# qinjr/SCoRe

Hardware: AMD Instinct MI355X
Metric: train samples/sec @ batch=1024 (higher is better)
Workload: dtype f32

## Files before the change

score_amd/csrc/engine.hip:

```cpp
#include <string.h>
#include <stdlib.h>
#include <stdio.h>
#include <math.h>
#include <mutex>
#include <new>
#include "common.h"
#include "kernels.h"
#include "persample.h"

namespace {

const int FC1 = 200, FC2 = 80, AT1 = 80, AT2 = 40;
const int CASER_L = SCORE_CASER_L, CASER_HPAD = SCORE_CASER_HPAD;
const int MAX_ENTRIES = 48;

enum Family { FAM_SLICE, FAM_GCMC, FAM_G4R, FAM_CASER, FAM_DELF, FAM_DEEMS, FAM_SVDPP, FAM_SASREC };

struct Dims {
  int64_t N;
  int D, H, T, K, Fu, Fi, mt;
  int Du, Di, I, Dq, NI, Dk, Dhead, nstate;
  int Is[2];
  bool coattn, attn;
  Family family;
  int n_gru;
  bool fc_head;
  bool sums_1hop;
  bool reads_targets;
  int Ic;
  int off_u, off_i, off_ti, off_tu;
};
// ... 221 lines not shown
static inline bool same_key(const LayoutKey& a, const LayoutKey& b) { return memcmp(&a, &b, sizeof(a)) == 0; }
int build_layout(const Dims& d, score_param_entry_t* out, int max_entries, Params* P) {
  struct Memo { bool ok; LayoutKey k; Params P; int n; score_param_entry_t ent[MAX_ENTRIES]; };
  static thread_local Memo memo = {};
  LayoutKey k = layout_key(d, 0);
  if (!memo.ok || !same_key(memo.k, k)) {
    memset(&memo.k, 0, sizeof(memo.k));
    memo.n = build_layout_raw(d, memo.ent, MAX_ENTRIES, &memo.P);
    memo.k = k; memo.ok = memo.n >= 0;
    if (memo.n < 0) return memo.n;
  }
  *P = memo.P;
  if (out) {
    if (memo.n > max_entries) return SCORE_E_BADARG;
    memcpy(out, memo.ent, sizeof(score_param_entry_t) * memo.n);
  }
  return memo.n;
}

struct WS {
  int64_t xside[2], info, rsave[2], query, head_inp, att_score, logit, y_pred, loss;
  int64_t gru_out[2], gru_final[2], xproj[2], gates[2];
  int64_t q, ainp, a1, a2, bn, f1, f2, lossb, dlogit, part;
  int64_t weff, wq, qz, adzsum, dweff, dwq, dqd;
  int64_t dwslab, dwslab_floats, dgstage, scratch2, gru_tmp, gru_tmp_floats;
  int64_t dz2, dz1, dbn, dhead, ds, da2, da1, dainp, dgru[2], dinfo, dq, dquery, dfinal[2];
  int64_t dxproj[2], rh[2], hprev[2], dxside[2], dzsum[2], S, scratch;
  int64_t pcoef[2], dzcoef[2], dtgt, keys_in, keys_out, vals_in, vals_out, sort_temp, partials;
  int64_t n_occ, sort_temp_bytes, partial_floats;
  int64_t uid, unique_rows, meta, remap[6];
  int64_t ca_slab, ca_slab_floats, cs_part, cs_part_floats, wxcat;
  int64_t pimg_x[2], pimg_d[2];
  int64_t psimg;
  int64_t gcmc_a[2], gcmc_z[2], gcmc_dz[2], gcmc_da[2], gcmc_pn, gcmc_g, gcmc_gu;
  int64_t caser_hwin, caser_arg, caser_v;
  int64_t delf_key[2], delf_att[2], delf_rep[2], delf_ds[2], delf_dpre[2], delf_act, delf_dact;
  int64_t deems_f1, deems_f2, deems_dz1, deems_dz2, deems_logit, deems_y, deems_dlogit;
  int64_t svdpp_act, svdpp_dw;
  int64_t sas_nrm, sas_qin, sas_q, sas_k, sas_v, sas_y, sas_dq, sas_dk, sas_dv, sas_rstd, sas_km, sas_p, sas_att, sas_fin,
      sas_dgamma, sas_dbeta, sas_hin, sas_dhin, sas_z1, sas_dz1, sas_f1, sas_dz1e, sas_z2, sas_f2, sas_dz2, sas_logit, sas_dlogit;
  int64_t scratch_floats, total;
};

static int panel_x_splits(int H) { return 3 * H <= 512 ? 1 : ((3 * H) % 32 == 0 && 3 * H <= 1024 ? 2 : 0); }
static int panel_d_splits(int I) { return I <= 512 ? 1 : (I % 32 == 0 && I <= 1024 ? 2 : 0); }

static int64_t ps_image_region_floats(const Dims& d) {
  if (d.H != 32 || !d.coattn || !d.attn) return 0;
  PsShape s;
  memset(&s, 0, sizeof(s));
  s.H = d.H; s.I = d.I; s.Dk = d.Dk; s.Dhead = d.Dhead;
  PsImages im;
  ps_plan_images(s, &im);
  return im.total;
}

static inline int64_t weff_copy_stride(const Dims& d) { return align_up64(2 * (int64_t)d.Dk * AT1 + 48, 4); }
struct Taker {
  int64_t cur;
  int64_t operator()(int64_t n) { int64_t o = cur; cur = align_up64(cur + (n > 0 ? n : 4), 4); return o; }
};
void ws_family_regions(const Dims& d, int B, Taker& take, WS* w) {
  const int64_t BT = (int64_t)B * d.T;
  if (d.family == FAM_GCMC) {
    const int Dx[2] = {d.Di, d.Du};
    for (int s = 0; s < 2; ++s) {
      w->gcmc_a[s] = take(BT * Dx[s]); w->gcmc_z[s] = take(BT * Dx[s]);
      w->gcmc_dz[s] = take(BT * Dx[s]); w->gcmc_da[s] = take(BT * Dx[s]);
    }
    w->gcmc_pn = take(2 * (int64_t)B * d.H); w->gcmc_g = take(B); w->gcmc_gu = take(2 * (int64_t)B * d.H);
  } else {
    for (int s = 0; s < 2; ++s) w->gcmc_a[s] = w->gcmc_z[s] = w->gcmc_dz[s] = w->gcmc_da[s] = -1;
    w->gcmc_pn = w->gcmc_g = w->gcmc_gu = -1;
  }
  if (d.family == FAM_CASER) {
    w->caser_hwin = take((int64_t)B * (d.T - CASER_L + 1)); w->caser_arg = take(B); w->caser_v = take((int64_t)B * d.Di);
  } else {
    w->caser_hwin = w->caser_arg = w->caser_v = -1;
  }
  if (d.family == FAM_DELF) {
// ... 31 lines not shown
  } else {
    w->sas_nrm = w->sas_qin = w->sas_q = w->sas_k = w->sas_v = w->sas_y = w->sas_dq = w->sas_dk = w->sas_dv = w->sas_rstd = w->sas_km =
        w->sas_p = w->sas_att = w->sas_fin = w->sas_dgamma = w->sas_dbeta = w->sas_hin = w->sas_dhin = w->sas_z1 = w->sas_dz1 = w->sas_f1 =
            w->sas_dz1e = w->sas_z2 = w->sas_f2 = w->sas_dz2 = w->sas_logit = w->sas_dlogit = -1;
  }
}

void build_ws_raw(const Dims& d, int B, WS* w) {
  Taker take = {0};
  const int64_t BT = (int64_t)B * d.T;
  for (int s = 0; s < 2; ++s) w->xside[s] = take(BT * d.I);
  w->info = take(BT * 4 * d.K);
  for (int c = 0; c < 2; ++c) w->rsave[c] = take(BT * d.K);
  w->query = take((int64_t)B * d.Dq);
  w->head_inp = take((int64_t)B * d.Dhead);
  w->att_score = take(BT);
  w->logit = take(B); w->y_pred = take(B); w->loss = take(4);
  for (int s = 0; s < 2; ++s) w->gru_out[s] = take(BT * d.H);
  for (int s = 0; s < 2; ++s) w->gru_final[s] = take((int64_t)B * d.H);
  for (int s = 0; s < 2; ++s) w->xproj[s] = take(BT * 3 * d.H);
  for (int s = 0; s < 2; ++s) w->gates[s] = take(BT * 3 * d.H);
  w->q = take((int64_t)B * d.Dk);
  w->ainp = take(BT * 2 * d.Dk);
  w->weff = take(SCORE_WEFF_COPIES * weff_copy_stride(d)); w->wq = take((int64_t)d.Dk * AT1); w->qz = take((int64_t)B * AT1);
  w->a1 = take(BT * AT1); w->a2 = take(BT * AT2);
  w->bn = take((int64_t)B * d.Dhead);
  w->f1 = take((int64_t)B * FC1); w->f2 = take((int64_t)B * FC2);
  w->lossb = take(B); w->dlogit = take(B); w->part = take(256 + 4);
  w->dz2 = take((int64_t)B * FC2); w->dz1 = take((int64_t)B * FC1);
  w->dbn = take((int64_t)B * d.Dhead); w->dhead = take((int64_t)B * d.Dhead);
  w->ds = take(BT); w->da2 = take(BT * AT2); w->da1 = take(BT * AT1);
  w->dainp = take(BT * 2 * d.Dk);
  w->adzsum = take((int64_t)B * AT1); w->dweff = take(2 * (int64_t)d.Dk * AT1); w->dwq = take((int64_t)d.Dk * AT1);
  w->dqd = take((int64_t)B * d.Dk);
  for (int s = 0; s < 2; ++s) w->dgru[s] = take(BT * d.H);
  w->dinfo = take(BT * 4 * d.K);
  w->dq = take((int64_t)B * d.Dk); w->dquery = take((int64_t)B * d.Dq);
  for (int s = 0; s < 2; ++s) w->dfinal[s] = take((int64_t)B * d.H);
  for (int s = 0; s < 2; ++s) {
    w->dxproj[s] = take(BT * 3 * d.H);
    w->rh[s] = take(BT * d.H);
    w->hprev[s] = take(BT * d.H + 3 * (int64_t)d.H * d.H);
  }
  for (int s = 0; s < 2; ++s) w->dxside[s] = take(BT * d.I);
  for (int c = 0; c < 2; ++c) w->dzsum[c] = take(BT);
  w->S = take(2 * (int64_t)B);
  w->scratch_floats = 4 << 20;
// ... 164 lines not shown
  return 0;
}

#define G(call) SCORE_TRY(call)
static inline int gemm_mode_call(int x3, int tr, int M, int N, int K, const float* A, int lda, const float* B,
                                 int ldb, float* C, int ldc, const float* bias, int flags, float keep,
                                 const uint8_t* mask, uint64_t seed, float* scratch, int64_t scratch_floats,
                                 void* s) {
  return score_gemm(tr, M, N, K, A, lda, B, ldb, C, ldc, bias, flags | x3, keep, mask, seed, scratch, scratch_floats,
                    s);
}
#define EV(i) \
  do { if (stage_events && stage_events[i]) HIPTRY(hipEventRecord((hipEvent_t)stage_events[i], s)); } while (0)

static inline uint32_t clamp_rows(int64_t n) { return (uint32_t)(n < 0x80000000ll ? n : 0x80000000ll); }
static inline int global_batch(const score_state_t* st, int B) { return st->global_batch > 0 ? st->global_batch : B; }

struct Pass {
  Dims d; Params P; WS w; Flags fl;
  const score_state_t* st; const score_batch_t* bt;
  int B, T, BT, H;
  int x3, Bg;
  uint32_t n_rows;
  int64_t weff_stride;
  float rs;
  float* ws; const float* W; float* scratch;
  hipStream_t s;
};
static int pass_fill(Pass* c, const score_state_t* st, const score_batch_t* bt, void* stream) {
  const Dims& d = c->d;
  build_layout(d, nullptr, 0, &c->P);
  c->st = st; c->bt = bt; c->fl = flags_of(st);
  c->B = bt->B; c->T = active_T(d, bt); c->H = d.H; c->BT = c->B * c->T;
  build_ws(d, c->B, &c->w);
  if (c->w.total * 4 > st->workspace_bytes) return SCORE_E_WORKSPACE;
  c->x3 = st->gemm_mode == 1 ? GF_X3 : 0; c->Bg = global_batch(st, c->B); c->n_rows = clamp_rows(st->n_table_rows);
  c->weff_stride = weff_copy_stride(d); c->rs = (float)(1.0 / sqrt(1.0 + 1e-3));
  c->ws = st->workspace; c->W = st->w; c->scratch = c->ws + c->w.scratch;
  c->s = (hipStream_t)stream;
  return 0;
}
static inline const float* wxcat(const Pass& c, int sd) { return c.ws + c.w.wxcat + (int64_t)sd * (c.d.Ic + 1) * 3 * c.H; }
static int weight_prep(const Pass& c, hipStream_t on) {
  const Dims& d = c.d; const Params& P = c.P; const WS& w = c.w; const float* W = c.W;
  return score_launch_weight_prep(W + P.gk[0], W + P.ck[0], W + P.gb[0], W + P.cb[0], W + P.gk[1], W + P.ck[1], W + P.gb[1],
                                  W + P.cb[1], d.Is[0], d.Is[1], d.Ic, d.H, c.ws + w.wxcat, d.Dk, AT1,
                                  d.attn ? W + P.at_w[1] : nullptr, c.ws + w.weff, c.ws + w.wq, SCORE_WEFF_COPIES, c.weff_stride, W,
                                  P.n_reg, c.ws + w.part, on);
}

static inline const float* gru_x_rows(const Pass& c, int sd) {
  return c.ws + (c.d.family == FAM_GCMC ? c.w.gcmc_z[sd] : (c.d.family == FAM_G4R && sd == 1) ? c.w.gru_out[0] : c.w.xside[sd]);
}

static void gru_header(const Pass& c, GruArgs* ga) {
  memset(ga, 0, sizeof(*ga));
  ga->B = c.B; ga->T = c.T; ga->H = c.H; ga->length = c.bt->length;
  ga->nw8 = 1;
  ga->tmp = c.ws + c.w.gru_tmp; ga->tmp_floats = c.w.gru_tmp_floats;
  ga->x3 = c.x3 != 0; ga->x3_rec = ga->x3 && !c.fl.gru_f32_rec; ga->stepwise = c.fl.gru_stepwise;
}
static void gru_side(const Pass& c, int sd, GruSide* g) {
  const int H = c.H;
  g->Wg = c.W + c.P.gk[sd] + (int64_t)c.d.Is[sd] * 2 * H; g->ldwg = 2 * H;
  g->Wc = c.W + c.P.ck[sd] + (int64_t)c.d.Is[sd] * H; g->ldwc = H;
  g->out = c.ws + c.w.gru_out[sd]; g->ldo = H; g->gates = c.ws + c.w.gates[sd];
}
static void gru_side_saved(const Pass& c, int sd, GruSide* g) {
  g->dxproj = c.ws + c.w.dxproj[sd]; g->rh = c.ws + c.w.rh[sd]; g->hprev = c.ws + c.w.hprev[sd];
}
// ... 825 lines not shown
      G(panel_launch(c, 0, xin, xp));
    } else {
      const float* Bx[2] = {wxcat(c, 0), wxcat(c, 1)};
      const float* bx[2] = {Bx[0] + (int64_t)d.Is[0] * 3 * H, Bx[1] + (int64_t)d.Is[1] * 3 * H};
      G(score_gemm_same_shape(0, 2, BT, 3 * H, d.Is[0], xin, x_ld(d, 0), Bx, 3 * H, xp, 3 * H, GF_BIAS, x3 != 0, c.scratch,
                              w.scratch_floats, s, bx));
    }
  }
  for (int sd = 0; sd < 2; ++sd) {
    const float* cat = wxcat(c, sd);
    if (d.Is[0] != d.Is[1])
      G(gemm_mode_call(x3, 0, BT, 3 * H, d.Is[sd], xin[sd], x_ld(d, sd), cat, 3 * H, xp[sd], 3 * H, cat + (int64_t)d.Is[sd] * 3 * H,
                       GF_BIAS, 1.f, nullptr, 0, c.scratch, w.scratch_floats, s));
    gru_side(c, sd, &ga.s[sd]);
    ga.s[sd].xproj = xp[sd]; ga.s[sd].final_state = ws + w.gru_final[sd];
  }
  return score_gru_fwd_multi(ga, 2, s);
}

int fwd_attention(const Pass& c, const FwdState& f) {
  const Dims& d = c.d; const Params& P = c.P; const WS& w = c.w; const score_batch_t* bt = c.bt;
  float* ws = c.ws; const float* W = c.W; const int B = c.B, T = c.T, H = c.H, BT = c.BT, x3 = c.x3; hipStream_t s = c.s;
  HIPTRY(hipStreamWaitEvent(s, f.sd->join, 0));
  int frc = c.fl.attn_unfused ? SCORE_E_SHAPE
                : score_launch_attn_fwd_fused(B, T, H, d.NI, AT1, AT2, ws + w.q, ws + w.gru_out[0], ws + w.gru_out[1],
                                              ws + w.info, ws + w.weff, ws + w.qz, W + P.at_w[2], W + P.at_b[2],
                                              W + P.at_w[3], W + P.at_b[3], bt->length, ws + w.ainp, ws + w.a1, ws + w.a2,
                                              ws + w.att_score, ws + w.head_inp, d.Dhead, d.off_u, d.off_i, s,
                                              SCORE_WEFF_COPIES, c.weff_stride);
  if (frc != SCORE_E_SHAPE) return frc;
  G(score_launch_attn_build_inp(B, T, H, d.NI, ws + w.q, ws + w.gru_out[0], ws + w.gru_out[1], ws + w.info,
                                ws + w.ainp, s));
  G(gemm_mode_call(x3, 0, BT, AT1, 2 * d.Dk, ws + w.ainp, 2 * d.Dk, ws + w.weff, AT1, ws + w.a1, AT1, ws + w.qz,
                   GF_BIAS | GF_RELU | (T << 16), 1.f, nullptr, 0, c.scratch, w.scratch_floats, s));
  int trc = c.fl.attn_unfused ? SCORE_E_SHAPE
                : score_launch_attn_tail_fwd(B, T, H, AT1, AT2, ws + w.a1, W + P.at_w[2], W + P.at_b[2], W + P.at_w[3],
                                             W + P.at_b[3], bt->length, ws + w.gru_out[0], ws + w.gru_out[1], ws + w.a2,
                                             ws + w.att_score, ws + w.head_inp, d.Dhead, d.off_u, d.off_i, s);
  if (trc != SCORE_E_SHAPE) return trc;
  G(gemm_mode_call(x3, 0, BT, AT2, AT1, ws + w.a1, AT1, W + P.at_w[2], AT2, ws + w.a2, AT2, W + P.at_b[2],
                   GF_BIAS | GF_RELU, 1.f, nullptr, 0, c.scratch, w.scratch_floats, s));
  return score_launch_attn_pool_fwd(B, T, H, AT2, ws + w.a2, W + P.at_w[3], W + P.at_b[3], bt->length,
                                    ws + w.gru_out[0], ws + w.gru_out[1], ws + w.att_score, ws + w.head_inp, d.Dhead,
                                    d.off_u, d.off_i, s);
}

int fwd_fc_head(const Pass& c, const FwdState& f) {
  const Dims& d = c.d; const Params& P = c.P; const WS& w = c.w; const score_state_t* st = c.st; const score_batch_t* bt = c.bt;
  float* ws = c.ws; const float* W = c.W; const int B = c.B, x3 = c.x3; hipStream_t s = c.s;
  const float keep_prob = f.keep_prob;
  const int dflag = keep_prob < 1.f ? GF_DROP : 0;
  int hrc = c.fl.head_unfused ? SCORE_E_SHAPE
// ... 664 lines not shown
```

score_amd/csrc/head.hip:

```cpp
#include <stdlib.h>
#include "common.h"
#include "kernels.h"
#include "cell.h"

__device__ __forceinline__ void attn_fold_w1_body(int blk, int Dk, int NA, const float* __restrict__ W1, float* __restrict__ weff,
                                                  float* __restrict__ wq, int copies, int64_t copy_stride) {
  int i = blk * 256 + threadIdx.x;
  if (i >= Dk * NA) return;
  const float wa = W1[i], wb = W1[Dk * NA + i], wc = W1[2 * Dk * NA + i], wd = W1[3 * Dk * NA + i];
  for (int c = 0; c < copies; ++c) {
    weff[c * copy_stride + i] = wb - wc;
    weff[c * copy_stride + Dk * NA + i] = wd;
  }
  wq[i] = wa + wc;
}

__global__ void attn_build_inp_kernel(int BT, int T, int H, int NI, const float* __restrict__ q,
                                      const float* __restrict__ ur, const float* __restrict__ ir,
                                      const float* __restrict__ info, float* __restrict__ inp) {
  const int Dk = 2 * H + NI;
  int64_t i = (int64_t)blockIdx.x * blockDim.x + threadIdx.x;
  if (i >= (int64_t)BT * Dk) return;
  int bt = (int)(i / Dk), j = (int)(i - (int64_t)bt * Dk);
  int b = bt / T;
  float k = j < H ? ur[(int64_t)bt * H + j]
                  : (j < 2 * H ? ir[(int64_t)bt * H + (j - H)] : info[(int64_t)bt * NI + (j - 2 * H)]);
  float qq = q[(int64_t)b * Dk + j];
  float* o = inp + (int64_t)bt * 2 * Dk;
  o[j] = k;
  o[Dk + j] = qq * k;
}
__global__ __launch_bounds__(256) void attn_build_inp4_kernel(int BT, int T, int H, int NI, const float* __restrict__ q,
                                                              const float* __restrict__ ur, const float* __restrict__ ir,
                                                              const float* __restrict__ info, float* __restrict__ inp) {
  const int Dk = 2 * H + NI, Dk4 = Dk >> 2;
  const unsigned i = blockIdx.x * blockDim.x + threadIdx.x;
  if (i >= (unsigned)BT * (unsigned)Dk4) return;
// ... 452 lines not shown
  const float* gk1; const float* ck1; const float* gb1; const float* cb1;
  int I0, I1, Imax, H; float* cat;
};
__device__ __forceinline__ void gru_wxcat_body(int blk, const WxcatArgs& a) {
  const int H = a.H;
  const int64_t per = (int64_t)(a.Imax + 1) * 3 * H;
  int64_t i = (int64_t)blk * 256 + threadIdx.x;
  if (i >= 2 * per) return;
  const int sd = i >= per;
  const int64_t l = i - sd * per;
  const int r = (int)(l / (3 * H)), j = (int)(l - (int64_t)r * 3 * H);
  const int I = sd ? a.I1 : a.I0;
  if (r > I) return;
  const float* gk = sd ? a.gk1 : a.gk0; const float* ck = sd ? a.ck1 : a.ck0;
  const float* gb = sd ? a.gb1 : a.gb0; const float* cb = sd ? a.cb1 : a.cb0;
  float v;
  if (r < I) v = j < 2 * H ? gk[(int64_t)r * 2 * H + j] : ck[(int64_t)r * H + (j - 2 * H)];
  else v = j < 2 * H ? gb[j] : cb[j - 2 * H];
  a.cat[i] = v;
}

struct WeightPrepArgs {
  WxcatArgs wx; int b_wx;
  int Dk, NA; const float* W1; float* weff; float* wq; int copies; int64_t copy_stride; int b_fold;
  const float* wreg; int64_t n_reg; float* part;
};
__global__ __launch_bounds__(256) void weight_prep_kernel(const WeightPrepArgs a) {
  const int b = blockIdx.x;
  if (b < a.b_wx) gru_wxcat_body(b, a.wx);
  else if (b < a.b_wx + a.b_fold) attn_fold_w1_body(b - a.b_wx, a.Dk, a.NA, a.W1, a.weff, a.wq, a.copies, a.copy_stride);
  else sumsq_stage1_body(b - a.b_wx - a.b_fold, L2_PARTS, a.wreg, a.n_reg, a.part);
}
int score_launch_weight_prep(const float* gk0, const float* ck0, const float* gb0, const float* cb0, const float* gk1,
                             const float* ck1, const float* gb1, const float* cb1, int I0, int I1, int Imax, int H, float* cat,
                             int Dk, int NA, const float* W1, float* weff, float* wq, int copies, int64_t copy_stride,
                             const float* wreg, int64_t n_reg, float* part, hipStream_t s) {
  WeightPrepArgs a;
  a.wx = WxcatArgs{gk0, ck0, gb0, cb0, gk1, ck1, gb1, cb1, I0, I1, Imax, H, cat};
  a.b_wx = (int)cdiv64(2 * (int64_t)(Imax + 1) * 3 * H, 256);
  a.Dk = Dk; a.NA = NA; a.W1 = W1; a.weff = weff; a.wq = wq; a.copies = copies; a.copy_stride = copy_stride;
  a.b_fold = W1 ? (Dk * NA + 255) / 256 : 0;
  a.wreg = wreg; a.n_reg = n_reg; a.part = part;
  hipLaunchKernelGGL(weight_prep_kernel, dim3(a.b_wx + a.b_fold + L2_PARTS), dim3(256), 0, s, a);
  SCORE_CHECK_LAUNCH();
  return 0;
}
#define adam1 score_adam1
__global__ void adam_kernel(float* __restrict__ p, float* __restrict__ m, float* __restrict__ v,
                            const float* __restrict__ g, int64_t n4, int64_t n, int64_t n_reg, float l2, float alpha,
                            float omb1, float omb2, float eps, const float* __restrict__ alpha_dev,
                            const int32_t* __restrict__ guard, int32_t* __restrict__ skipped) {
  if (guard && *guard) {
    if (skipped && blockIdx.x == 0 && threadIdx.x == 0) atomicAdd(skipped, 1);
    return;
  }
  if (alpha_dev) alpha = *alpha_dev;
  score_adam_dense_body(p, m, v, g, n4, n, n_reg, l2, alpha, omb1, omb2, eps, (int)blockIdx.x, (int)gridDim.x);
}

#ifndef ADAM_NT
#define ADAM_NT 0
#endif
__device__ __forceinline__ float4 adam_ld(const float* p) {
#if ADAM_NT
  const score_v4f t = __builtin_nontemporal_load(reinterpret_cast<const score_v4f*>(p));
  return make_float4(t.x, t.y, t.z, t.w);
// ... 222 lines not shown
```

score_amd/csrc/head_fused.hip:

```cpp
#include "common.h"
#include "kernels.h"
#include "cell.h"
#include "head_tiles.h"

namespace {

struct HeadFwdArgs {
  int B, Dh, N1, N2, Bglobal;
  const float* x; const float* gamma; const float* beta; float rs;
  const float* W1; const float* b1; const float* W2; const float* b2; const float* W3; const float* b3;
  float keep; int drop; const uint8_t* mask0; const uint8_t* mask1; uint64_t seed0, seed1;
  const uint64_t* seed_dev;
  const int32_t* label;
  float* bn; float* f1; float* f2; float* logit; float* y; float* lossb; float* dlogit;
  float* dz2;
  int phase;
};

__global__ __launch_bounds__(64 * HF_NW) void head_fwd_fused_kernel(const HeadFwdArgs a) {
  extern __shared__ float sm[];
  const uint64_t seed0 = a.seed_dev ? *a.seed_dev : a.seed0;
  const uint64_t seed1 = a.seed_dev ? (seed0 ^ 0x5DEECE66Dull) : a.seed1;
  const int Dh = a.Dh, N1 = a.N1, N2 = a.N2;
  const int Kp0 = (Dh + 15) & ~15, LD0 = Kp0 + 4;
  const int Kp1 = (N1 + 15) & ~15, LD1 = Kp1 + 4;
  const int Kp2 = (N2 + 15) & ~15, LD2 = Kp2 + 4;
// ... 138 lines not shown
      a.y[row] = p;
      a.lossb[row] = logloss_term(p, lab);
      const float dl = logloss_dlogit(p, lab, a.Bglobal);
      a.dlogit[row] = dl;
      xs[i] = dl;
    }
  }
  __syncthreads();
  if (a.dz2) {
    for (int e = tid; e < HF_ROWS * N2; e += 64 * HF_NW) {
      const int i = e / N2, n = e - i * N2, row = b0 + i;
      const float q = xs[i] * a.W3[n] / a.keep;
      if (row < a.B) a.dz2[(int64_t)row * N2 + n] = f2s[i * LD2 + n] > 0.f ? q : 0.f;
    }
  }
}


constexpr int AF_NW = 8;

struct AttnFwdArgs {
  int B, T, H, NI, N1, N2, S;
  const float* q; const float* ur; const float* ir; const float* info;
  const float* Weff; const float* qz;
  const float* W4; const float* b4; const float* w5; const float* b5; const int32_t* length;
  float* inp; float* a1; float* a2; float* score; float* head; int ldh, off_u, off_i;
  int wcopies; int64_t wstride;
};

__device__ __forceinline__ void af_build(const AttnFwdArgs& a, float* __restrict__ xs, int LD, int Kp, int row0,
                                         int row_end, int t0, int nthr) {
  const int Dk = 2 * a.H + a.NI, Dk4 = Dk >> 2, K2 = 2 * Dk;
  const int total = 16 * Dk4;
  constexpr int U = 4;
  for (int e0 = t0; e0 < total; e0 += U * nthr) {
    float4 k[U], qq[U];
    int ii[U], jj[U], gg[U];
    bool ok[U];
#pragma unroll
    for (int u = 0; u < U; ++u) {
      const int e = e0 + u * nthr;
      const int ec = e < total ? e : 0;
      ii[u] = ec / Dk4; jj[u] = (ec - ii[u] * Dk4) * 4;
      gg[u] = row0 + ii[u];
      ok[u] = e < total && gg[u] < row_end;
      const int g = gg[u] < row_end ? gg[u] : row_end - 1;
      const int j = jj[u];
      const float* src = j < a.H ? a.ur + (int64_t)g * a.H + j
                                 : (j < 2 * a.H ? a.ir + (int64_t)g * a.H + (j - a.H) : a.info + (int64_t)g * a.NI + (j - 2 * a.H));
      k[u] = ld4(src);
// ... 10 lines not shown
#endif
      } else {
        kk = make_float4(0.f, 0.f, 0.f, 0.f); qk = kk;
      }
      *reinterpret_cast<float4*>(xs + ii[u] * LD + jj[u]) = kk;
      *reinterpret_cast<float4*>(xs + ii[u] * LD + Dk + jj[u]) = qk;
    }
  }
  for (int e = t0; e < 16 * (Kp - K2); e += nthr) {
    const int i = e / (Kp - K2), j = e - i * (Kp - K2);
    xs[i * LD + K2 + j] = 0.f;
  }
}

template <int KQ>
__global__ __launch_bounds__(64 * AF_NW) void attn_fwd_fused_kernel(const AttnFwdArgs a) {
  extern __shared__ float sm[];
  const int T = a.T, H = a.H, N1 = a.N1, N2 = a.N2;
  const int Dk = 2 * H + a.NI, K2 = 2 * Dk, Kp = 4 * KQ, LD = Kp + 4;
  const int L1 = N1 + 1, L2 = N2 + 1;
  float* xs0 = sm;
  float* xs1 = xs0 + 16 * LD;
  float* a1s = xs1 + 16 * LD;
  float* w4s = a1s + a.S * T * L1;
  float* a2s = w4s + N1 * N2;
  float* scs = a2s + a.S * T * L2;
  const int tid = threadIdx.x, lane = tid & 63, wave = tid >> 6;
  const int lc = lane & 15, lq = lane >> 4;
  const int b0 = blockIdx.x * a.S;
  const int ns = min(a.S, a.B - b0);
  const int row0 = b0 * T, row_end = row0 + ns * T;
  const int ntile = (ns * T + 15) >> 4;
  const int ntn = (N1 + 15) >> 4;

  float breg[KQ];
  if (wave < ntn) {
    const int col = wave * 16 + lc;
    const float* Wsrc = a.Weff + (int64_t)((blockIdx.x >> 3) % a.wcopies) * a.wstride;
#pragma unroll
    for (int s_ = 0; s_ < KQ; ++s_) {
      const int k = lq * KQ + s_;
#ifdef AFP_NOPRELOAD
      const float w = (float)(k + col) * 1e-3f;
#else
      const float w = Wsrc[(int64_t)(k < K2 ? k : K2 - 1) * N1 + (col < N1 ? col : N1 - 1)];
#endif
      breg[s_] = w * ((k < K2 && col < N1) ? 1.0f : 0.0f);
    }
  }
  for (int i = tid; i < N1 * N2; i += 64 * AF_NW) w4s[i] = a.W4[i];
  af_build(a, xs0, LD, Kp, row0, row_end, tid, 64 * AF_NW);
  __syncthreads();
  for (int m = 0; m < ntile; ++m) {
    float* xs = (m & 1) ? xs1 : xs0;
    if (wave < ntn) {
      hf_f32x4 acc[1] = {{0.f, 0.f, 0.f, 0.f}};
      const int n0[1] = {wave * 16};
      const float* xrow = xs + lc * LD + lq * KQ;
#ifndef AFP_NOMFMA
#ifdef AFP_TWOACC
      hf_f32x4 acc2 = {0.f, 0.f, 0.f, 0.f};
#pragma unroll
      for (int s4 = 0; s4 < KQ; s4 += 4) {
        const float4 av = *reinterpret_cast<const float4*>(xrow + s4);
        acc[0] = __builtin_amdgcn_mfma_f32_16x16x4f32(av.x, breg[s4 + 0], acc[0], 0, 0, 0);
        acc2 = __builtin_amdgcn_mfma_f32_16x16x4f32(av.y, breg[s4 + 1], acc2, 0, 0, 0);
        acc[0] = __builtin_amdgcn_mfma_f32_16x16x4f32(av.z, breg[s4 + 2], acc[0], 0, 0, 0);
        acc2 = __builtin_amdgcn_mfma_f32_16x16x4f32(av.w, breg[s4 + 3], acc2, 0, 0, 0);
      }
      acc[0] += acc2;
// ... 27 lines not shown
#endif
          }
        }
      }
    } else if (m + 1 < ntile) {
#ifndef AFP_NOBUILD
      af_build(a, (m & 1) ? xs0 : xs1, LD, Kp, row0 + (m + 1) * 16, row_end, tid - 64 * ntn, 64 * (AF_NW - ntn));
#endif
    }
    __syncthreads();
  }

#ifdef AFP_NOTAIL
  return;
#endif
  const int gsz = 64 * AF_NW / a.S, s_ = tid / gsz, gt = tid - s_ * gsz;
  const bool live = s_ < ns;
  const int b = b0 + (live ? s_ : 0);
  const float* a1b = a1s + s_ * T * L1;
  float* a2l = a2s + s_ * T * L2;
  float* sc = scs + s_ * T;
  if (live) {
    float* a2b = a.a2 + (int64_t)b * T * N2;
    for (int i = gt; i < T * N2; i += gsz) {
      const int t = i / N2, n = i - t * N2;
      float acc = 0.f;
#pragma unroll 8
      for (int k = 0; k < N1; ++k) acc = fmaf(a1b[t * L1 + k], w4s[k * N2 + n], acc);
      const float v = fmaxf(acc + a.b4[n], 0.f);
      a2l[t * L2 + n] = v;
      a2b[i] = v;
    }
  }
  __syncthreads();
  if (live) {
    const int len = a.length[b];
    for (int t = gt; t < T; t += gsz) {
      float acc = 0.f;
      for (int n = 0; n < N2; ++n) acc = fmaf(a2l[t * L2 + n], a.w5[n], acc);
      sc[t] = t < len ? acc + a.b5[0] : -4294967295.0f;
    }
  }
  __syncthreads();
  float mx = -INFINITY, den = 0.f;
  if (live) {
    for (int t = 0; t < T; ++t) mx = fmaxf(mx, sc[t]);
    for (int t = 0; t < T; ++t) den += expf(sc[t] - mx);
  }
  __syncthreads();
  if (live) {
    for (int t = gt; t < T; t += gsz) {
      const float v = expf(sc[t] - mx) / den;
      sc[t] = v;
      a.score[(int64_t)b * T + t] = v;
// ... 248 lines not shown
  a.x = x; a.gamma = gamma; a.beta = beta; a.rs = rs;
  a.W1 = W1; a.b1 = b1; a.W2 = W2; a.b2 = b2; a.W3 = W3; a.b3 = b3;
  a.keep = keep; a.drop = keep < 1.f ? 1 : 0; a.mask0 = mask0; a.mask1 = mask1; a.seed0 = seed0; a.seed1 = seed1; a.seed_dev = seed_dev;
  a.label = label; a.bn = bn; a.f1 = f1; a.f2 = f2; a.logit = logit; a.y = y; a.lossb = lossb; a.dlogit = dlogit;
  a.dz2 = dz2;
  const int mt = (B + HF_ROWS - 1) / HF_ROWS, nt1 = (N1 + 15) >> 4;
  const bool split = !single_launch && nt1 >= 4 && mt >= 32;
  if (!split) {
    a.phase = 0;
    hipLaunchKernelGGL(head_fwd_fused_kernel, dim3(mt), dim3(64 * HF_NW), lds, s, a);
    SCORE_CHECK_LAUNCH();
    return 0;
  }
  a.phase = 1;
  hipLaunchKernelGGL(head_fwd_fused_kernel, dim3(mt, 4), dim3(64 * HF_NW), lds, s, a);
  SCORE_CHECK_LAUNCH();
  a.phase = 2;
  hipLaunchKernelGGL(head_fwd_fused_kernel, dim3(mt), dim3(64 * HF_NW), lds, s, a);
  SCORE_CHECK_LAUNCH();
  return 0;
}

int score_launch_attn_fwd_fused(int B, int T, int H, int NI, int N1, int N2, const float* q, const float* ur,
                                const float* ir, const float* info, const float* Weff, const float* qz, const float* W4,
                                const float* b4, const float* w5, const float* b5, const int32_t* length, float* inp,
                                float* a1, float* a2, float* score, float* head, int ldh, int off_u, int off_i,
                                hipStream_t s, int weff_copies, int64_t weff_copy_stride) {
  if (B <= 0 || T <= 0 || (H & 3) || (NI & 3) || N1 > 16 * 5 || N1 <= 0 || N2 <= 0 || (int64_t)B * T >= (1LL << 30))
    return SCORE_E_SHAPE;
  const int K2 = 2 * (2 * H + NI), Kp = (K2 + 15) & ~15, LD = Kp + 4;
  int S = B >= 4 * 256 ? 4 : B >= 2 * 256 ? 2 : 1;
  size_t lds = 0;
  for (; S >= 1; S >>= 1) {
    lds = ((size_t)2 * 16 * LD + (size_t)S * T * (N1 + 1) + (size_t)N1 * N2 + (size_t)S * T * (N2 + 1) + (size_t)S * T) * sizeof(float);
    if (lds <= 150 * 1024) break;
  }
  if (S < 1) return SCORE_E_SHAPE;
  const int kq = Kp / 4;
  if (kq != 148 && kq != 52 && kq != 44 && kq != 36 && kq != 84) return SCORE_E_SHAPE;
  static thread_local bool attr_set = false;
  if (!attr_set) {
    for (const void* f : {reinterpret_cast<const void*>(attn_fwd_fused_kernel<148>),
                          reinterpret_cast<const void*>(attn_fwd_fused_kernel<52>),
                          reinterpret_cast<const void*>(attn_fwd_fused_kernel<44>),
                          reinterpret_cast<const void*>(attn_fwd_fused_kernel<36>),
                          reinterpret_cast<const void*>(attn_fwd_fused_kernel<84>)}) {
      hipError_t e = hipFuncSetAttribute(f, hipFuncAttributeMaxDynamicSharedMemorySize, 150 * 1024);
      if (e != hipSuccess) return (int)e;
    }
    attr_set = true;
  }
  AttnFwdArgs a;
  a.B = B; a.T = T; a.H = H; a.NI = NI; a.N1 = N1; a.N2 = N2; a.S = S;
  a.q = q; a.ur = ur; a.ir = ir; a.info = info; a.Weff = Weff; a.qz = qz;
  a.W4 = W4; a.b4 = b4; a.w5 = w5; a.b5 = b5; a.length = length;
  a.inp = inp; a.a1 = a1; a.a2 = a2; a.score = score; a.head = head; a.ldh = ldh; a.off_u = off_u; a.off_i = off_i;
  a.wcopies = weff_copies > 0 ? weff_copies : 1; a.wstride = weff_copy_stride;
  const dim3 grid((B + S - 1) / S), block(64 * AF_NW);
  switch (Kp / 4) {
    case 148: hipLaunchKernelGGL(attn_fwd_fused_kernel<148>, grid, block, lds, s, a); break;
    case 52: hipLaunchKernelGGL(attn_fwd_fused_kernel<52>, grid, block, lds, s, a); break;
    case 44: hipLaunchKernelGGL(attn_fwd_fused_kernel<44>, grid, block, lds, s, a); break;
    case 36: hipLaunchKernelGGL(attn_fwd_fused_kernel<36>, grid, block, lds, s, a); break;
    case 84: hipLaunchKernelGGL(attn_fwd_fused_kernel<84>, grid, block, lds, s, a); break;
    default: return SCORE_E_SHAPE;
  }
  SCORE_CHECK_LAUNCH();
  return 0;
}

static bool ab_plan(int B, int T, int H, int NI, int N1, int N2, int ldh, int off_u, int off_i, bool pool, int* S_out,
                    size_t* lds_out) {
  const int Dk = 2 * H + NI, K2 = 2 * Dk;
  if (B <= 0 || T <= 0 || (H & 3) || (NI & 3) || N1 != 4 * AB_KQ || K2 > 16 * AF_NW * AB_NTW || (int64_t)B * T >= (1LL << 30) ||
      (ldh & 3) || (off_u >= 0 && (off_u & 3)) || (off_i >= 0 && (off_i & 3)) || (pool && N2 <= 0))
    return false;
  const int S = B >= 4 * 256 ? 4 : B >= 2 * 256 ? 2 : 1;
  const int RT = ((S * T + 15) >> 4) << 4;
  const size_t lds = ((size_t)RT * (N1 + 4) + (size_t)16 * (K2 + 4) + (size_t)S * Dk +
                      (pool ? (size_t)S * T + (size_t)S * T * (N2 + 1) + (size_t)N1 * (N2 + 1) : 0)) * sizeof(float);
  if (lds > 150 * 1024) return false;
  *S_out = S; *lds_out = lds;
  return true;
}
bool score_attn_inp_bwd_fused_fits(int B, int T, int H, int NI, int N1, int N2, int ldh, int off_u, int off_i, bool pool) {
  int S; size_t lds;
  return ab_plan(B, T, H, NI, N1, N2, ldh, off_u, off_i, pool, &S, &lds);
}

// ... 41 lines not shown
```

score_amd/csrc/kernels.h:

```cpp
#pragma once
#include "common.h"

#define GEMM_GROUP_MAX 16
struct GemmProb {
  const float* A; const float* B; float* C; float* slab;
  const float* bias;
  int M, N, K, lda, ldb, ldc, k_chunk, gx, gy, nblocks;
};
struct GemmGroup { int n; int total_blocks; GemmProb p[GEMM_GROUP_MAX]; };
enum { GF_BIAS = 1, GF_RELU = 2, GF_ACC = 4, GF_DROP = 8, GF_X3 = 16, GF_X3F = 32, GF_RELUGRAD = 64 };
__device__ __forceinline__ int64_t bias_index(int flags, int row, int col, int N) {
  const int g = flags >> 16;
  return g ? (int64_t)(row / g) * N + col : col;
}
__device__ __forceinline__ float gemm_epilogue(float v, int row, int col, int N, const float* bias, int flags,
                                               float keep, const uint8_t* mask, uint64_t seed) {
  if (flags & GF_BIAS) v += bias[bias_index(flags, row, col, N)];
  if (flags & GF_RELU) v = fmaxf(v, 0.f);
  if (flags & GF_DROP) {
    uint64_t e = (uint64_t)row * (uint64_t)N + (uint64_t)col;
    bool on = mask ? (mask[e] != 0) : (hash_uniform(seed, e) < keep);
    v = on ? v / keep : 0.f;
  }
  if (flags & GF_RELUGRAD) {
// ... 62 lines not shown
                                const float* info, float* inp, hipStream_t s);
int score_launch_attn_pool_fwd(int B, int T, int H, int NA, const float* a2, const float* w5, const float* b5,
                               const int32_t* length, const float* ur, const float* ir, float* score, float* head,
                               int ldh, int off_u, int off_i, hipStream_t s);
int score_launch_attn_tail_fwd(int B, int T, int H, int N1, int N2, const float* a1, const float* W4, const float* b4,
                               const float* w5, const float* b5, const int32_t* length, const float* ur, const float* ir,
                               float* a2, float* score, float* head, int ldh, int off_u, int off_i, hipStream_t s);
int score_launch_attn_pool_bwd(int B, int T, int H, int NA, const float* a2, const float* w5,
                               const int32_t* length, const float* ur, const float* ir, const float* score,
                               const float* dhead, int ldh, int off_u, int off_i, float* ds, float* da2,
                               hipStream_t s, int N1 = 0, const float* W4 = nullptr, const float* a1 = nullptr,
                               float* da1 = nullptr);
int score_launch_attn_inp_bwd(int B, int T, int H, int NI, const float* dinp, const float* q, const float* ur,
                              const float* ir, const float* info, const float* score, const float* dhead, int ldh,
                              int off_u, int off_i, const float* dqd, float* dur, float* dir, float* dinfo, float* dq,
                              hipStream_t s);
int score_launch_attn_inp_bwd_fused(int B, int T, int H, int NI, int N1, const float* da1, const float* Weff, const float* q,
                                    const float* ur, const float* ir, const float* info, const float* score,
                                    const float* dhead, int ldh, int off_u, int off_i, float* dur, float* dir, float* dinfo,
                                    float* dq, hipStream_t s, int N2 = 0, const float* a2 = nullptr, const float* a1 = nullptr,
                                    const float* w5 = nullptr, const float* W4 = nullptr, const int32_t* length = nullptr,
                                    float* ds = nullptr, float* da2 = nullptr, float* da1_out = nullptr);
bool score_attn_inp_bwd_fused_fits(int B, int T, int H, int NI, int N1, int N2, int ldh, int off_u, int off_i, bool pool);
#define SCORE_WEFF_COPIES 8
int score_launch_attn_dzsum(int B, int T, int NA, const float* dz, float* dzsum, hipStream_t s);
int score_launch_attn_w1_grad(int Dk, int NA, const float* dweff, const float* dwq, float* gW1, hipStream_t s);
int score_launch_bn_fwd(int B, int Dh, const float* x, const float* gamma, const float* beta, float rs, float* y,
                        hipStream_t s);
int score_launch_bn_bwd(int B, int Dh, const float* x, const float* gamma, float rs, const float* dy, float* dx,
                        float* dgamma, float* dbeta, float* tmp, float* scratch, int64_t scratch_floats,
                        ColsumJobs* cq, hipStream_t s);
int score_launch_weight_prep(const float* gk0, const float* ck0, const float* gb0, const float* cb0, const float* gk1,
                             const float* ck1, const float* gb1, const float* cb1, int I0, int I1, int Imax, int H, float* cat,
                             int Dk, int NA, const float* W1, float* weff, float* wq, int copies, int64_t copy_stride,
                             const float* wreg, int64_t n_reg, float* part, hipStream_t s);
int score_launch_head_out(int B, int NF, const float* f2, const float* w3, const float* b3, const int32_t* label,
                          float* logit, float* y, float* lossb, float* dlogit, float* loss, float lambda,
                          const float* part, int Bglobal, hipStream_t s, const int32_t* id_status = nullptr);
int score_launch_loss_final(int B, const float* lossb, float* loss, float lambda, const float* part, int Bglobal,
                            hipStream_t s, const int32_t* id_status = nullptr);
int score_launch_head_fwd_fused(int B, int Dh, int N1, int N2, const float* x, const float* gamma, const float* beta,
                                float rs, const float* W1, const float* b1, const float* W2, const float* b2,
                                const float* W3, const float* b3, float keep, const uint8_t* mask0, const uint8_t* mask1,
                                uint64_t seed0, uint64_t seed1, const int32_t* label, float* bn, float* f1, float* f2,
                                float* logit, float* y, float* lossb, float* dlogit, int Bglobal, hipStream_t s,
                                const uint64_t* seed_dev = nullptr, float* dz2 = nullptr, int single_launch = 0);
bool score_head_fwd_fused_fits(int B, int Dh, int N1, int N2);
int score_launch_head_bwd_fused(int B, int Dh, int N1, int N2, const float* dz2, const float* W2, const float* f1, float keep,
                                const float* W1, const float* x, const float* gamma, float rs, float* dz1, float* dbn,
                                float* dhead, float* tmp, hipStream_t s);
int score_launch_attn_fwd_fused(int B, int T, int H, int NI, int N1, int N2, const float* q, const float* ur,
                                const float* ir, const float* info, const float* Weff, const float* qz, const float* W4,
                                const float* b4, const float* w5, const float* b5, const int32_t* length, float* inp,
                                float* a1, float* a2, float* score, float* head, int ldh, int off_u, int off_i,
                                hipStream_t s, int weff_copies = 1, int64_t weff_copy_stride = 0);
int score_launch_outer_relu_bwd(int B, int NF, const float* dlogit, const float* w, const float* f, float keep,
                                float* dz, hipStream_t s);
int score_launch_copy2d(int64_t rows, int cols, const float* src, int lds_, float* dst, int ldd, hipStream_t s);

struct PlanFillArgs {
  const int32_t* idx[6];
  int64_t off[7];
  int F[6];
  int K, G, shift;
  int T, TA;
  uint32_t n_rows;
  int32_t* id_status;
};
struct PullArgs {
  const float* G[6]; int ldg[6]; int gcol[6];
  const float* cA[6]; const float* cB[6];
  const float* Wv[6];
  float constA[6];
  const uint32_t* uid;
  int D, K, LPRp;
  int zero_is_dummy;
  uint8_t* flags;
};
// ... 155 lines not shown
```

Before: 921,400.

## Prepack attention Weff into per-lane float4 image and vectorize a2 layer

Replaces the eight replicated copies of the folded attention weight with a single register-image layout, written once during weight prep. Each lane of the fused attention forward kernel can then preload its B-fragment with coalesced float4 loads instead of strided scalar gathers with bounds masking. The second attention layer (a2) is also vectorized over four output columns using float4 LDS reads and stores, with a small LDS alignment pad. This costs an extra image-building pass in weight prep and adds alignment requirements that, if unmet, send the code to the unfused path.

After: 927,300, median of 6. No clear change (+0.6%).

```diff
diff --git a/score_amd/csrc/attn_image.h b/score_amd/csrc/attn_image.h
--- /dev/null
+++ b/score_amd/csrc/attn_image.h
@@ -0,0 +1,20 @@
+#pragma once
+#include "common.h"
+
+#define SCORE_ATTN_NB 5
+
+static inline int64_t score_attn_image_floats(int K) { return (int64_t)SCORE_ATTN_NB * (((K + 15) & ~15) / 4) * 64; }
+
+template <class F>
+__device__ __forceinline__ void attn_image_body(int64_t i, int N, int K, F wt, float4* __restrict__ img) {
+  const int KQ = ((K + 15) & ~15) / 4;
+  if (i >= (int64_t)SCORE_ATTN_NB * (KQ / 4) * 64) return;
+  const int lane = (int)(i & 63);
+  const int64_t ts = i >> 6;
+  const int s4 = (int)(ts % (KQ / 4)), t = (int)(ts / (KQ / 4));
+  const int n = t * 16 + (lane & 15), k0 = (lane >> 4) * KQ + 4 * s4;
+  float v[4];
+#pragma unroll
+  for (int e = 0; e < 4; ++e) v[e] = (n < N && k0 + e < K) ? wt(n, k0 + e) : 0.f;
+  img[i] = make_float4(v[0], v[1], v[2], v[3]);
+}
diff --git a/score_amd/csrc/engine.hip b/score_amd/csrc/engine.hip
--- a/score_amd/csrc/engine.hip
+++ b/score_amd/csrc/engine.hip
@@ -7,6 +7,7 @@
 #include "common.h"
 #include "kernels.h"
 #include "persample.h"
+#include "attn_image.h"
 
 namespace {
 
@@ -274,7 +275,7 @@
   int64_t xside[2], info, rsave[2], query, head_inp, att_score, logit, y_pred, loss;
   int64_t gru_out[2], gru_final[2], xproj[2], gates[2];
   int64_t q, ainp, a1, a2, bn, f1, f2, lossb, dlogit, part;
-  int64_t weff, wq, qz, adzsum, dweff, dwq, dqd;
+  int64_t weff, weff_img, wq, qz, adzsum, dweff, dwq, dqd;
   int64_t dwslab, dwslab_floats, dgstage, scratch2, gru_tmp, gru_tmp_floats;
   int64_t dz2, dz1, dbn, dhead, ds, da2, da1, dainp, dgru[2], dinfo, dq, dquery, dfinal[2];
   int64_t dxproj[2], rh[2], hprev[2], dxside[2], dzsum[2], S, scratch;
@@ -307,7 +308,10 @@
   return im.total;
 }
 
-static inline int64_t weff_copy_stride(const Dims& d) { return align_up64(2 * (int64_t)d.Dk * AT1 + 48, 4); }
+static inline int64_t weff_slot_stride(const Dims& d) { return align_up64(2 * (int64_t)d.Dk * AT1 + 48, 4); }
+static inline int64_t weff_image_offset(const Dims& d) {
+  return d.Dk > 0 && score_attn_image_floats(2 * d.Dk) <= 7 * weff_slot_stride(d) ? weff_slot_stride(d) : -1;
+}
 struct Taker {
   int64_t cur;
   int64_t operator()(int64_t n) { int64_t o = cur; cur = align_up64(cur + (n > 0 ? n : 4), 4); return o; }
@@ -385,7 +389,7 @@
   for (int s = 0; s < 2; ++s) w->gates[s] = take(BT * 3 * d.H);
   w->q = take((int64_t)B * d.Dk);
   w->ainp = take(BT * 2 * d.Dk);
-  w->weff = take(SCORE_WEFF_COPIES * weff_copy_stride(d)); w->wq = take((int64_t)d.Dk * AT1); w->qz = take((int64_t)B * AT1);
+  w->weff = take(8 * weff_slot_stride(d)); w->weff_img = weff_image_offset(d) < 0 ? -1 : w->weff + weff_image_offset(d); w->wq = take((int64_t)d.Dk * AT1); w->qz = take((int64_t)B * AT1);
   w->a1 = take(BT * AT1); w->a2 = take(BT * AT2);
   w->bn = take((int64_t)B * d.Dhead);
   w->f1 = take((int64_t)B * FC1); w->f2 = take((int64_t)B * FC2);
@@ -596,7 +600,6 @@
   int B, T, BT, H;
   int x3, Bg;
   uint32_t n_rows;
-  int64_t weff_stride;
   float rs;
   float* ws; const float* W; float* scratch;
   hipStream_t s;
@@ -609,7 +612,7 @@
   build_ws(d, c->B, &c->w);
   if (c->w.total * 4 > st->workspace_bytes) return SCORE_E_WORKSPACE;
   c->x3 = st->gemm_mode == 1 ? GF_X3 : 0; c->Bg = global_batch(st, c->B); c->n_rows = clamp_rows(st->n_table_rows);
-  c->weff_stride = weff_copy_stride(d); c->rs = (float)(1.0 / sqrt(1.0 + 1e-3));
+  c->rs = (float)(1.0 / sqrt(1.0 + 1e-3));
   c->ws = st->workspace; c->W = st->w; c->scratch = c->ws + c->w.scratch;
   c->s = (hipStream_t)stream;
   return 0;
@@ -619,7 +622,7 @@
   const Dims& d = c.d; const Params& P = c.P; const WS& w = c.w; const float* W = c.W;
   return score_launch_weight_prep(W + P.gk[0], W + P.ck[0], W + P.gb[0], W + P.cb[0], W + P.gk[1], W + P.ck[1], W + P.gb[1],
                                   W + P.cb[1], d.Is[0], d.Is[1], d.Ic, d.H, c.ws + w.wxcat, d.Dk, AT1,
-                                  d.attn ? W + P.at_w[1] : nullptr, c.ws + w.weff, c.ws + w.wq, SCORE_WEFF_COPIES, c.weff_stride, W,
+                                  d.attn ? W + P.at_w[1] : nullptr, c.ws + w.weff, c.ws + w.wq, w.weff_img < 0 ? nullptr : c.ws + w.weff_img, W,
                                   P.n_reg, c.ws + w.part, on);
 }
 
@@ -1491,12 +1494,11 @@
   const Dims& d = c.d; const Params& P = c.P; const WS& w = c.w; const score_batch_t* bt = c.bt;
   float* ws = c.ws; const float* W = c.W; const int B = c.B, T = c.T, H = c.H, BT = c.BT, x3 = c.x3; hipStream_t s = c.s;
   HIPTRY(hipStreamWaitEvent(s, f.sd->join, 0));
-  int frc = c.fl.attn_unfused ? SCORE_E_SHAPE
+  int frc = c.fl.attn_unfused || w.weff_img < 0 ? SCORE_E_SHAPE
                 : score_launch_attn_fwd_fused(B, T, H, d.NI, AT1, AT2, ws + w.q, ws + w.gru_out[0], ws + w.gru_out[1],
-                                              ws + w.info, ws + w.weff, ws + w.qz, W + P.at_w[2], W + P.at_b[2],
+                                              ws + w.info, ws + w.weff_img, ws + w.qz, W + P.at_w[2], W + P.at_b[2],
                                               W + P.at_w[3], W + P.at_b[3], bt->length, ws + w.ainp, ws + w.a1, ws + w.a2,
-                                              ws + w.att_score, ws + w.head_inp, d.Dhead, d.off_u, d.off_i, s,
-                                              SCORE_WEFF_COPIES, c.weff_stride);
+                                              ws + w.att_score, ws + w.head_inp, d.Dhead, d.off_u, d.off_i, s);
   if (frc != SCORE_E_SHAPE) return frc;
   G(score_launch_attn_build_inp(B, T, H, d.NI, ws + w.q, ws + w.gru_out[0], ws + w.gru_out[1], ws + w.info,
                                 ws + w.ainp, s));
diff --git a/score_amd/csrc/head.hip b/score_amd/csrc/head.hip
--- a/score_amd/csrc/head.hip
+++ b/score_amd/csrc/head.hip
@@ -2,17 +2,21 @@
 #include "common.h"
 #include "kernels.h"
 #include "cell.h"
+#include "attn_image.h"
 
 __device__ __forceinline__ void attn_fold_w1_body(int blk, int Dk, int NA, const float* __restrict__ W1, float* __restrict__ weff,
-                                                  float* __restrict__ wq, int copies, int64_t copy_stride) {
+                                                  float* __restrict__ wq) {
   int i = blk * 256 + threadIdx.x;
   if (i >= Dk * NA) return;
   const float wa = W1[i], wb = W1[Dk * NA + i], wc = W1[2 * Dk * NA + i], wd = W1[3 * Dk * NA + i];
-  for (int c = 0; c < copies; ++c) {
-    weff[c * copy_stride + i] = wb - wc;
-    weff[c * copy_stride + Dk * NA + i] = wd;
-  }
+  weff[i] = wb - wc;
+  weff[Dk * NA + i] = wd;
   wq[i] = wa + wc;
+}
+__device__ __forceinline__ void attn_weff_image_body(int blk, int Dk, int NA, const float* __restrict__ W1, float4* __restrict__ img) {
+  const int DN = Dk * NA;
+  attn_image_body((int64_t)blk * 256 + threadIdx.x, NA, 2 * Dk,
+                  [&](int n, int k) { return k < Dk ? W1[DN + k * NA + n] - W1[2 * DN + k * NA + n] : W1[3 * DN + (k - Dk) * NA + n]; }, img);
 }
 
 __global__ void attn_build_inp_kernel(int BT, int T, int H, int NI, const float* __restrict__ q,
@@ -511,26 +515,29 @@
 
 struct WeightPrepArgs {
   WxcatArgs wx; int b_wx;
-  int Dk, NA; const float* W1; float* weff; float* wq; int copies; int64_t copy_stride; int b_fold;
+  int Dk, NA; const float* W1; float* weff; float* wq; float4* weff_img; int b_fold, b_img;
   const float* wreg; int64_t n_reg; float* part;
 };
 __global__ __launch_bounds__(256) void weight_prep_kernel(const WeightPrepArgs a) {
   const int b = blockIdx.x;
   if (b < a.b_wx) gru_wxcat_body(b, a.wx);
-  else if (b < a.b_wx + a.b_fold) attn_fold_w1_body(b - a.b_wx, a.Dk, a.NA, a.W1, a.weff, a.wq, a.copies, a.copy_stride);
-  else sumsq_stage1_body(b - a.b_wx - a.b_fold, L2_PARTS, a.wreg, a.n_reg, a.part);
+  else if (b < a.b_wx + a.b_fold) attn_fold_w1_body(b - a.b_wx, a.Dk, a.NA, a.W1, a.weff, a.wq);
+  else if (b < a.b_wx + a.b_fold + a.b_img) attn_weff_image_body(b - a.b_wx - a.b_fold, a.Dk, a.NA, a.W1, a.weff_img);
+  else sumsq_stage1_body(b - a.b_wx - a.b_fold - a.b_img, L2_PARTS, a.wreg, a.n_reg, a.part);
 }
 int score_launch_weight_prep(const float* gk0, const float* ck0, const float* gb0, const float* cb0, const float* gk1,
                              const float* ck1, const float* gb1, const float* cb1, int I0, int I1, int Imax, int H, float* cat,
-                             int Dk, int NA, const float* W1, float* weff, float* wq, int copies, int64_t copy_stride,
+                             int Dk, int NA, const float* W1, float* weff, float* wq, float* weff_img,
                              const float* wreg, int64_t n_reg, float* part, hipStream_t s) {
   WeightPrepArgs a;
   a.wx = WxcatArgs{gk0, ck0, gb0, cb0, gk1, ck1, gb1, cb1, I0, I1, Imax, H, cat};
   a.b_wx = (int)cdiv64(2 * (int64_t)(Imax + 1) * 3 * H, 256);
-  a.Dk = Dk; a.NA = NA; a.W1 = W1; a.weff = weff; a.wq = wq; a.copies = copies; a.copy_stride = copy_stride;
+  if (W1 && weff_img && NA > 16 * SCORE_ATTN_NB) return SCORE_E_SHAPE;
+  a.Dk = Dk; a.NA = NA; a.W1 = W1; a.weff = weff; a.wq = wq; a.weff_img = reinterpret_cast<float4*>(weff_img);
   a.b_fold = W1 ? (Dk * NA + 255) / 256 : 0;
+  a.b_img = W1 && weff_img ? (int)cdiv64(score_attn_image_floats(2 * Dk) / 4, 256) : 0;
   a.wreg = wreg; a.n_reg = n_reg; a.part = part;
-  hipLaunchKernelGGL(weight_prep_kernel, dim3(a.b_wx + a.b_fold + L2_PARTS), dim3(256), 0, s, a);
+  hipLaunchKernelGGL(weight_prep_kernel, dim3(a.b_wx + a.b_fold + a.b_img + L2_PARTS), dim3(256), 0, s, a);
   SCORE_CHECK_LAUNCH();
   return 0;
 }
diff --git a/score_amd/csrc/head_fused.hip b/score_amd/csrc/head_fused.hip
--- a/score_amd/csrc/head_fused.hip
+++ b/score_amd/csrc/head_fused.hip
@@ -2,6 +2,7 @@
 #include "kernels.h"
 #include "cell.h"
 #include "head_tiles.h"
+#include "attn_image.h"
 
 namespace {
 
@@ -186,10 +187,9 @@
 struct AttnFwdArgs {
   int B, T, H, NI, N1, N2, S;
   const float* q; const float* ur; const float* ir; const float* info;
-  const float* Weff; const float* qz;
+  const float4* wimg; const float* qz;
   const float* W4; const float* b4; const float* w5; const float* b5; const int32_t* length;
   float* inp; float* a1; float* a2; float* score; float* head; int ldh, off_u, off_i;
-  int wcopies; int64_t wstride;
 };
 
 __device__ __forceinline__ void af_build(const AttnFwdArgs& a, float* __restrict__ xs, int LD, int Kp, int row0,
@@ -246,7 +246,7 @@
   float* xs0 = sm;
   float* xs1 = xs0 + 16 * LD;
   float* a1s = xs1 + 16 * LD;
-  float* w4s = a1s + a.S * T * L1;
+  float* w4s = a1s + ((a.S * T * L1 + 3) & ~3);
   float* a2s = w4s + N1 * N2;
   float* scs = a2s + a.S * T * L2;
   const int tid = threadIdx.x, lane = tid & 63, wave = tid >> 6;
@@ -259,17 +259,15 @@
 
   float breg[KQ];
   if (wave < ntn) {
-    const int col = wave * 16 + lc;
-    const float* Wsrc = a.Weff + (int64_t)((blockIdx.x >> 3) % a.wcopies) * a.wstride;
-#pragma unroll
-    for (int s_ = 0; s_ < KQ; ++s_) {
-      const int k = lq * KQ + s_;
+    const float4* img = a.wimg + (size_t)wave * (KQ / 4) * 64 + lane;
+#pragma unroll
+    for (int s4 = 0; s4 < KQ / 4; ++s4) {
 #ifdef AFP_NOPRELOAD
-      const float w = (float)(k + col) * 1e-3f;
+      const float4 w = make_float4((float)(s4 + lane) * 1e-3f, 0.f, 1e-3f, 2e-3f);
 #else
-      const float w = Wsrc[(int64_t)(k < K2 ? k : K2 - 1) * N1 + (col < N1 ? col : N1 - 1)];
+      const float4 w = img[s4 * 64];
 #endif
-      breg[s_] = w * ((k < K2 && col < N1) ? 1.0f : 0.0f);
+      breg[4 * s4 + 0] = w.x; breg[4 * s4 + 1] = w.y; breg[4 * s4 + 2] = w.z; breg[4 * s4 + 3] = w.w;
     }
   }
   for (int i = tid; i < N1 * N2; i += 64 * AF_NW) w4s[i] = a.W4[i];
@@ -343,14 +341,28 @@
   float* sc = scs + s_ * T;
   if (live) {
     float* a2b = a.a2 + (int64_t)b * T * N2;
-    for (int i = gt; i < T * N2; i += gsz) {
-      const int t = i / N2, n = i - t * N2;
-      float acc = 0.f;
+    if ((N2 & 3) == 0) {
+      const int N4 = N2 >> 2;
+      for (int i = gt; i < T * N4; i += gsz) {
+        const int t = i / N4, n = (i - t * N4) * 4;
+        float4 acc = make_float4(0.f, 0.f, 0.f, 0.f);
 #pragma unroll 8
-      for (int k = 0; k < N1; ++k) acc = fmaf(a1b[t * L1 + k], w4s[k * N2 + n], acc);
-      const float v = fmaxf(acc + a.b4[n], 0.f);
-      a2l[t * L2 + n] = v;
-      a2b[i] = v;
+        for (int k = 0; k < N1; ++k) acc = fma4(a1b[t * L1 + k], *reinterpret_cast<const float4*>(w4s + k * N2 + n), acc);
+        const float4 bb = make_float4(a.b4[n], a.b4[n + 1], a.b4[n + 2], a.b4[n + 3]);
+        const float4 v = make_float4(fmaxf(acc.x + bb.x, 0.f), fmaxf(acc.y + bb.y, 0.f), fmaxf(acc.z + bb.z, 0.f), fmaxf(acc.w + bb.w, 0.f));
+        a2l[t * L2 + n] = v.x; a2l[t * L2 + n + 1] = v.y; a2l[t * L2 + n + 2] = v.z; a2l[t * L2 + n + 3] = v.w;
+        st4(a2b + t * N2 + n, v);
+      }
+    } else {
+      for (int i = gt; i < T * N2; i += gsz) {
+        const int t = i / N2, n = i - t * N2;
+        float acc = 0.f;
+#pragma unroll 8
+        for (int k = 0; k < N1; ++k) acc = fmaf(a1b[t * L1 + k], w4s[k * N2 + n], acc);
+        const float v = fmaxf(acc + a.b4[n], 0.f);
+        a2l[t * L2 + n] = v;
+        a2b[i] = v;
+      }
     }
   }
   __syncthreads();
@@ -645,17 +657,18 @@
 }
 
 int score_launch_attn_fwd_fused(int B, int T, int H, int NI, int N1, int N2, const float* q, const float* ur,
-                                const float* ir, const float* info, const float* Weff, const float* qz, const float* W4,
+                                const float* ir, const float* info, const float* Weff_img, const float* qz, const float* W4,
                                 const float* b4, const float* w5, const float* b5, const int32_t* length, float* inp,
                                 float* a1, float* a2, float* score, float* head, int ldh, int off_u, int off_i,
-                                hipStream_t s, int weff_copies, int64_t weff_copy_stride) {
-  if (B <= 0 || T <= 0 || (H & 3) || (NI & 3) || N1 > 16 * 5 || N1 <= 0 || N2 <= 0 || (int64_t)B * T >= (1LL << 30))
+                                hipStream_t s) {
+  if (B <= 0 || T <= 0 || (H & 3) || (NI & 3) || N1 > 16 * SCORE_ATTN_NB || N1 <= 0 || N2 <= 0 || (int64_t)B * T >= (1LL << 30) ||
+      ((uintptr_t)Weff_img & 15) || ((uintptr_t)a2 & 15))
     return SCORE_E_SHAPE;
   const int K2 = 2 * (2 * H + NI), Kp = (K2 + 15) & ~15, LD = Kp + 4;
   int S = B >= 4 * 256 ? 4 : B >= 2 * 256 ? 2 : 1;
   size_t lds = 0;
   for (; S >= 1; S >>= 1) {
-    lds = ((size_t)2 * 16 * LD + (size_t)S * T * (N1 + 1) + (size_t)N1 * N2 + (size_t)S * T * (N2 + 1) + (size_t)S * T) * sizeof(float);
+    lds = ((size_t)2 * 16 * LD + (size_t)S * T * (N1 + 1) + 3 + (size_t)N1 * N2 + (size_t)S * T * (N2 + 1) + (size_t)S * T) * sizeof(float);
     if (lds <= 150 * 1024) break;
   }
   if (S < 1) return SCORE_E_SHAPE;
@@ -675,10 +688,9 @@
   }
   AttnFwdArgs a;
   a.B = B; a.T = T; a.H = H; a.NI = NI; a.N1 = N1; a.N2 = N2; a.S = S;
-  a.q = q; a.ur = ur; a.ir = ir; a.info = info; a.Weff = Weff; a.qz = qz;
+  a.q = q; a.ur = ur; a.ir = ir; a.info = info; a.wimg = reinterpret_cast<const float4*>(Weff_img); a.qz = qz;
   a.W4 = W4; a.b4 = b4; a.w5 = w5; a.b5 = b5; a.length = length;
   a.inp = inp; a.a1 = a1; a.a2 = a2; a.score = score; a.head = head; a.ldh = ldh; a.off_u = off_u; a.off_i = off_i;
-  a.wcopies = weff_copies > 0 ? weff_copies : 1; a.wstride = weff_copy_stride;
   const dim3 grid((B + S - 1) / S), block(64 * AF_NW);
   switch (Kp / 4) {
     case 148: hipLaunchKernelGGL(attn_fwd_fused_kernel<148>, grid, block, lds, s, a); break;
@@ -688,6 +700,18 @@
     case 84: hipLaunchKernelGGL(attn_fwd_fused_kernel<84>, grid, block, lds, s, a); break;
     default: return SCORE_E_SHAPE;
   }
+  SCORE_CHECK_LAUNCH();
+  return 0;
+}
+
+__global__ __launch_bounds__(256) static void attn_weff_image_kernel(int K2, int N1, const float* __restrict__ Weff, float4* __restrict__ img) {
+  attn_image_body((int64_t)blockIdx.x * 256 + threadIdx.x, N1, K2, [&](int n, int k) { return Weff[(int64_t)k * N1 + n]; }, img);
+}
+int score_launch_attn_weff_image(int K2, int N1, const float* Weff, float* img, hipStream_t s) {
+  if (K2 <= 0 || N1 <= 0 || N1 > 16 * SCORE_ATTN_NB || ((uintptr_t)img & 15)) return SCORE_E_SHAPE;
+  const int64_t threads = score_attn_image_floats(K2) / 4;
+  hipLaunchKernelGGL(attn_weff_image_kernel, dim3((unsigned)((threads + 255) / 256)), dim3(256), 0, s, K2, N1, Weff,
+                     reinterpret_cast<float4*>(img));
   SCORE_CHECK_LAUNCH();
   return 0;
 }
diff --git a/score_amd/csrc/kernels.h b/score_amd/csrc/kernels.h
--- a/score_amd/csrc/kernels.h
+++ b/score_amd/csrc/kernels.h
@@ -108,7 +108,6 @@
                                     const float* w5 = nullptr, const float* W4 = nullptr, const int32_t* length = nullptr,
                                     float* ds = nullptr, float* da2 = nullptr, float* da1_out = nullptr);
 bool score_attn_inp_bwd_fused_fits(int B, int T, int H, int NI, int N1, int N2, int ldh, int off_u, int off_i, bool pool);
-#define SCORE_WEFF_COPIES 8
 int score_launch_attn_dzsum(int B, int T, int NA, const float* dz, float* dzsum, hipStream_t s);
 int score_launch_attn_w1_grad(int Dk, int NA, const float* dweff, const float* dwq, float* gW1, hipStream_t s);
 int score_launch_bn_fwd(int B, int Dh, const float* x, const float* gamma, const float* beta, float rs, float* y,
@@ -118,7 +117,7 @@
                         ColsumJobs* cq, hipStream_t s);
 int score_launch_weight_prep(const float* gk0, const float* ck0, const float* gb0, const float* cb0, const float* gk1,
                              const float* ck1, const float* gb1, const float* cb1, int I0, int I1, int Imax, int H, float* cat,
-                             int Dk, int NA, const float* W1, float* weff, float* wq, int copies, int64_t copy_stride,
+                             int Dk, int NA, const float* W1, float* weff, float* wq, float* weff_img,
                              const float* wreg, int64_t n_reg, float* part, hipStream_t s);
 int score_launch_head_out(int B, int NF, const float* f2, const float* w3, const float* b3, const int32_t* label,
                           float* logit, float* y, float* lossb, float* dlogit, float* loss, float lambda,
@@ -136,10 +135,11 @@
                                 const float* W1, const float* x, const float* gamma, float rs, float* dz1, float* dbn,
                                 float* dhead, float* tmp, hipStream_t s);
 int score_launch_attn_fwd_fused(int B, int T, int H, int NI, int N1, int N2, const float* q, const float* ur,
-                                const float* ir, const float* info, const float* Weff, const float* qz, const float* W4,
+                                const float* ir, const float* info, const float* Weff_img, const float* qz, const float* W4,
                                 const float* b4, const float* w5, const float* b5, const int32_t* length, float* inp,
                                 float* a1, float* a2, float* score, float* head, int ldh, int off_u, int off_i,
-                                hipStream_t s, int weff_copies = 1, int64_t weff_copy_stride = 0);
+                                hipStream_t s);
+int score_launch_attn_weff_image(int K2, int N1, const float* Weff, float* img, hipStream_t s);
 int score_launch_outer_relu_bwd(int B, int NF, const float* dlogit, const float* w, const float* f, float keep,
                                 float* dz, hipStream_t s);
 int score_launch_copy2d(int64_t rows, int cols, const float* src, int lds_, float* dst, int ldd, hipStream_t s);
```
